# khiner/MeshEditor

Hardware: AMD Instinct MI355X
Metric: eigenpairs/sec (K/M assembly + 50-mode solve, 100k-tet mesh) (higher is better)
Workload: dtype f64; 1 GPU; cube_s100k: Kuhn mesh 105456 tets / 446631 DOF, NumModes=50 NumFemModes=65, P=10 excitation points, one mesh per GPU; eigenpairs_per_mesh=65, kept_modes_per_mesh=50, parallelism=mesh-per-gpu x1

## Files before the change

### mesheditor_amd/csrc/mh_common.h

```cpp
#pragma once
#include "../../include/modalhip.h"

#include <hip/hip_runtime.h>
#include <rocblas/rocblas.h>
#include <rocsolver/rocsolver.h>

#include <algorithm>
#include <cstdarg>
#include <cstdio>
#include <cstdlib>
#include <cstring>
#include <iterator>
#include <limits>
#include <map>
#include <mutex>
#include <stdexcept>
#include <string>
#include <vector>

struct MhError : std::runtime_error {
    int code;
    MhError(int c, const std::string &m) : std::runtime_error(m), code(c) {}
};

// ... 491 lines not shown
    enum Solver { SYEVD = 0, SMALL_PARTIAL = 1, SMALL_STEDC = 2, WIDE_PARTIAL = 3, WIDE_STEDC_ORMTR = 4 };
    int reduction{-1};
    double defect{-1};
    int solver{-1};
    double quality{std::numeric_limits<double>::quiet_NaN()};
};
int mh_rr_solve(mh_context *ctx, double *gA, double *gM, uint32_t m, double *evals, double *ework, DevArray<int> &info, uint32_t nwant = 0, bool gm_is_identity = false,
                std::vector<double> *host_evals = nullptr);
void mh_spd_inverse_small(mh_context *ctx, const double *a, uint32_t lda, uint32_t w, double *out, uint32_t ldo, int *info);
void mh_potrf(mh_context *ctx, double *a, uint32_t ld, uint32_t w, int *info);
void mh_potrf_small(mh_context *ctx, double *a, uint32_t w, int *info);
void mh_potrf_small_inverse(mh_context *ctx, double *a, uint32_t w, int *info, const double *dscale, double *linv);
bool mh_sytrd_gave_up(mh_context *ctx);
void mh_sytrd_wide(mh_context *ctx, double *a, uint32_t m, double *d, double *e, double *tau);
void mh_sytrd_small(mh_context *ctx, double *a, uint32_t m, double *d, double *e, double *tau, int variant = -1);
void mh_small_gemm(mh_context *ctx, bool ta, bool tb, uint32_t M, uint32_t N, uint32_t K, double alpha, const double *a, uint32_t lda, const double *b, uint32_t ldb, double beta, double *c,
                   uint32_t ldc);
void mh_short_product(mh_context *ctx, size_t n, const double *a, uint32_t m, const double *ct, uint32_t nc, double *out, double *partial, uint32_t slices);
void mh_pack_stacked(mh_context *ctx, const double *c1, uint32_t r1, const double *c2, uint32_t r2, uint32_t cols, double scale, double *ct);
void mh_pack_coefficients(mh_context *ctx, const double *c1, uint32_t n1, const double *c2, uint32_t n2, uint32_t m, uint32_t ld, double *ct);
void mh_spmm_mapped(mh_context *ctx, const BsrLevel &lvl, const double *vals9, const double *x, double *y, const double *mscal, double *y2, uint32_t w, uint32_t ldy,
                    uint32_t wreal, const uint32_t *omap, const double *res_theta = nullptr, double *res_out = nullptr, double *res_partial = nullptr,
                    const double *res_dinv = nullptr);
bool mh_spmm_f32_cheb_step(mh_context *ctx, const BsrLevel &lvl, const float *d_in, float *d_out, float *r, float *x, const float *dinv, float c1, float c2,
                           uint32_t w);
void mh_spmm_f32(mh_context *ctx, const BsrLevel &lvl, const float *x, float *y, uint32_t w);
void mh_spmm_mixed(mh_context *ctx, const BsrLevel &lvl, const float *x, double *y, uint32_t w);
const uint32_t *mh_identity_map(mh_context *ctx);
void mh_spmm(mh_context *ctx, const BsrLevel &lvl, const double *vals9, const double *x, double *y, const double *mscal, double *y2, uint32_t w);
```

### mesheditor_amd/csrc/mh_eigs.hip

```cpp
#include "mh_common.h"

#include <algorithm>
#include <cmath>
#include <memory>
#include <condition_variable>
#include <mutex>
#include <numeric>
#include <optional>
#include <type_traits>

__global__ void k_shift_values(const double *kval, const double *mval, size_t nblocks, double sigma, double *aval);
__global__ void k_diag_inverse(const uint32_t *row_ptr, const uint32_t *col, const double *aval, uint32_t nnodes, double *dinv);
__global__ void k_coarse_matrix(const uint32_t *row_ptr, const uint32_t *col, const double *aval, const double *tmat, const uint32_t *agg_of, const uint32_t *agg_ptr,
                                const uint32_t *agg_nodes, uint32_t nagg, double *a0);
__global__ void k_fix_coarse_diag(double *a0, uint32_t n0, double rel);

namespace {
constexpr int TB = 256;

std::mutex g_solve_mutex;
struct Switches {
    bool verbose = getenv("MH_VERBOSE") != nullptr;
    bool fp32_prec = !(getenv("MH_PRECOND_FP64") && atoi(getenv("MH_PRECOND_FP64")) != 0);
    int deg2 = 0, deg1 = 0, gamma = 0;
    double cheb_ratio = 0.0, cheb_ratio1 = 0.0;
    bool test_sytrd_giveup = getenv("MH_TEST") && strstr(getenv("MH_TEST"), "sytrd_giveup");
    bool no_tridiag_wide = getenv("MH_TEST") && strstr(getenv("MH_TEST"), "no_tridiag_wide");
    bool test_last_resort = getenv("MH_TEST") && strstr(getenv("MH_TEST"), "last_resort");
    bool test_coarse_pivot = getenv("MH_TEST") && strstr(getenv("MH_TEST"), "coarse_pivot");
    bool test_selfcheck_fail = getenv("MH_TEST") && strstr(getenv("MH_TEST"), "selfcheck_fail");
    bool lmax_low = getenv("MH_TEST") && strstr(getenv("MH_TEST"), "lmax_low");
    bool potrf_chain = getenv("MH_TEST") && strstr(getenv("MH_TEST"), "potrf_chain");
    bool no_poly_start = getenv("MH_TEST") && strstr(getenv("MH_TEST"), "no_poly_start");
    Switches() {
        if (const char *c = getenv("MH_CYCLE")) {
            double v[5] = {0, 0, 0, 0, 0};
            sscanf(c, "%lf,%lf,%lf,%lf,%lf", &v[0], &v[1], &v[2], &v[3], &v[4]);
            deg2 = std::max(0, int(v[0])), deg1 = std::max(0, int(v[1])), gamma = std::max(0, int(v[2]));
            cheb_ratio = v[3];
            cheb_ratio1 = v[4];
        }
    }
};
const Switches &switches() {
    static const Switches s;
    return s;
}
constexpr int kPowerIterations = 20;
constexpr uint32_t kPrecondColumns = 256;
constexpr uint32_t kSkipP = 4;
constexpr uint32_t kGuardPercent = 10;
constexpr float kFlatShape = 1e-4f;
constexpr size_t kDenseLastResort = 12288;
constexpr int kLastResortCg = 8;

struct PhaseLock {
// ... 71 lines not shown
};

__global__ void k_random_panel(double *__restrict__ x, size_t count, uint64_t seed) {
    const size_t i = size_t(blockIdx.x) * blockDim.x + threadIdx.x;
    if (i >= count) return;
    auto mix = [](uint64_t z) {
        z += 0x9e3779b97f4a7c15ull;
        z = (z ^ (z >> 30)) * 0xbf58476d1ce4e5b9ull;
        z = (z ^ (z >> 27)) * 0x94d049bb133111ebull;
        return z ^ (z >> 31);
    };
    const uint64_t a = mix(seed + 2 * i), b = mix(seed + 2 * i + 1);
    const double u1 = (double(a >> 11) + 1.0) * (1.0 / 9007199254740993.0), u2 = double(b >> 11) * (1.0 / 9007199254740992.0);
    x[i] = sqrt(-2.0 * log(u1)) * cos(6.283185307179586 * u2);
}

template<typename T>
__global__ void k_cheb_init(const T *__restrict__ b, const T *__restrict__ t, const T *__restrict__ dinv, T inv_theta, T *__restrict__ r, T *__restrict__ d,
                            T *__restrict__ x, int accumulate, size_t rows, uint32_t w) {
    const size_t i = size_t(blockIdx.x) * blockDim.x + threadIdx.x;
    if (i >= rows * w) return;
    const T rv = t ? b[i] - t[i] : b[i];
    const T dv = dinv[i / w] * rv * inv_theta;
    r[i] = rv;
    d[i] = dv;
    x[i] = accumulate ? x[i] + dv : dv;
}
typedef float f4_t __attribute__((ext_vector_type(4)));
__global__ void k_cheb_init_v4(const f4_t *__restrict__ b, const f4_t *__restrict__ t, const float *__restrict__ dinv, float inv_theta, f4_t *__restrict__ r,
                               f4_t *__restrict__ d, f4_t *__restrict__ x, int accumulate, size_t rows, uint32_t w4) {
    const size_t i = size_t(blockIdx.x) * blockDim.x + threadIdx.x;
    if (i >= rows * w4) return;
    const f4_t rv = t ? b[i] - t[i] : b[i];
    const f4_t dv = (dinv[i / w4] * inv_theta) * rv;
    r[i] = rv;
    d[i] = dv;
    x[i] = accumulate ? x[i] + dv : dv;
}
__global__ void k_cheb_last_v4(const f4_t *__restrict__ t, const float *__restrict__ dinv, float c1, float c2, const f4_t *__restrict__ r, const f4_t *__restrict__ d,
                               const f4_t *__restrict__ x, double *__restrict__ z, size_t rows, uint32_t w4, uint32_t wo) {
    const size_t i = size_t(blockIdx.x) * blockDim.x + threadIdx.x;
    if (i >= rows * w4) return;
    const size_t row = i / w4;
    const uint32_t c = uint32_t(i % w4) * 4;
    const f4_t rv = r[i] - t[i];
    const f4_t zv = x[i] + (c1 * d[i] + (c2 * dinv[row]) * rv);
#pragma unroll
    for (int e = 0; e < 4; ++e)
        if (c + e < wo) z[row * wo + c + e] = double(zv[e]);
}
__global__ void k_prolong_p1_v4(const f4_t *__restrict__ x1, const uint32_t *__restrict__ pa, const uint32_t *__restrict__ pb, f4_t *__restrict__ x2, uint32_t nnodes,
                                uint32_t w4) {
    const size_t i = size_t(blockIdx.x) * blockDim.x + threadIdx.x;
    if (i >= size_t(nnodes) * 3 * w4) return;
    const uint32_t c = uint32_t(i % w4), comp = uint32_t((i / w4) % 3), node = uint32_t(i / (size_t(3) * w4));
    const uint32_t a = pa[node], bb = pb[node];
    const f4_t va = x1[(size_t(3) * a + comp) * w4 + c];
    x2[i] += a == bb ? va : 0.5f * (va + x1[(size_t(3) * bb + comp) * w4 + c]);
}
__global__ void k_cheb_init_convert(const double *__restrict__ src, uint32_t ws, const float *__restrict__ dinv, float inv_theta, float *__restrict__ b32,
                                    float *__restrict__ r, float *__restrict__ d, float *__restrict__ x, size_t rows, uint32_t w) {
    const size_t i = size_t(blockIdx.x) * blockDim.x + threadIdx.x;
    if (i >= rows * w) return;
    const size_t row = i / w;
    const uint32_t c = uint32_t(i % w);
    const float rv = c < ws ? float(src[row * ws + c]) : 0.f;
    const float dv = dinv[row] * rv * inv_theta;
    b32[i] = rv;
    r[i] = rv;
    d[i] = dv;
    x[i] = dv;
}
template<typename T>
__global__ void k_cheb_step(const T *__restrict__ t, const T *__restrict__ dinv, T c1, T c2, T *__restrict__ r, T *__restrict__ d, T *__restrict__ x, size_t rows,
                            uint32_t w) {
    const size_t i = size_t(blockIdx.x) * blockDim.x + threadIdx.x;
    if (i >= rows * w) return;
    const T rv = r[i] - t[i];
    const T dv = c1 * d[i] + c2 * dinv[i / w] * rv;
    r[i] = rv;
    d[i] = dv;
    x[i] += dv;
}
template<typename T>
__global__ void k_cheb_last(const T *__restrict__ t, const T *__restrict__ dinv, T c1, T c2, const T *__restrict__ r, const T *__restrict__ d, const T *__restrict__ x,
                            double *__restrict__ z, size_t rows, uint32_t w, uint32_t wo) {
    const size_t i = size_t(blockIdx.x) * blockDim.x + threadIdx.x;
    if (i >= rows * w) return;
    const size_t row = i / w;
    const uint32_t c = uint32_t(i % w);
    if (c >= wo) return;
    const T rv = r[i] - t[i];
    z[row * wo + c] = double(x[i] + (c1 * d[i] + c2 * dinv[row] * rv));
}
template<typename S, typename D> __global__ void k_convert(const S *__restrict__ src, D *__restrict__ dst, size_t count) {
    const size_t i = size_t(blockIdx.x) * blockDim.x + threadIdx.x;
    if (i < count) dst[i] = D(src[i]);
}
template<typename S, typename D> __global__ void k_convert_pitch(const S *__restrict__ src, uint32_t ws, D *__restrict__ dst, uint32_t wd, size_t rows) {
    const size_t i = size_t(blockIdx.x) * blockDim.x + threadIdx.x;
    if (i >= rows * wd) return;
    const size_t row = i / wd;
    const uint32_t c = uint32_t(i % wd);
    dst[i] = c < ws ? D(src[row * ws + c]) : D(0);
}

template<typename T>
__global__ void k_restrict_p1(const T *__restrict__ b, const T *__restrict__ t, const uint32_t *__restrict__ p1_corner, const uint32_t *__restrict__ eptr,
                              const uint32_t *__restrict__ emid, T *__restrict__ r1, uint32_t npts, uint32_t w, uint32_t wb = 0) {
    const size_t i = size_t(blockIdx.x) * blockDim.x + threadIdx.x;
    if (i >= size_t(npts) * 3 * w) return;
    const uint32_t c = uint32_t(i % w), comp = uint32_t((i / w) % 3), p = uint32_t(i / (size_t(3) * w));
    const uint32_t pb = wb ? wb : w;
    auto res = [&](uint32_t node) {
        const size_t row = size_t(3) * node + comp;
        return (c < pb ? b[row * pb + c] : T(0)) - t[row * w + c];
    };
    T s = res(p1_corner[p]);
    T h = 0;
    for (uint32_t e = eptr[p]; e < eptr[p + 1]; ++e) h += res(emid[e]);
    r1[i] = s + T(0.5) * h;
}
template<typename T>
__global__ void k_prolong_p1(const T *__restrict__ x1, const uint32_t *__restrict__ pa, const uint32_t *__restrict__ pb, T *__restrict__ x2, uint32_t nnodes,
                             uint32_t w) {
    const size_t i = size_t(blockIdx.x) * blockDim.x + threadIdx.x;
    if (i >= size_t(nnodes) * 3 * w) return;
    const uint32_t c = uint32_t(i % w), comp = uint32_t((i / w) % 3), node = uint32_t(i / (size_t(3) * w));
    const uint32_t a = pa[node], bb = pb[node];
    const T va = x1[(size_t(3) * a + comp) * w + c];
    x2[i] += a == bb ? va : T(0.5) * (va + x1[(size_t(3) * bb + comp) * w + c]);
}
template<typename T>
__global__ void k_restrict_agg(const T *__restrict__ b, const T *__restrict__ t, const double *__restrict__ tmat, double *__restrict__ r0,
                               const uint32_t *__restrict__ agg_ptr, const uint32_t *__restrict__ agg_nodes, uint32_t nagg, uint32_t w) {
    const size_t i = size_t(blockIdx.x) * blockDim.x + threadIdx.x;
    if (i >= size_t(nagg) * 6 * w) return;
    const uint32_t c = uint32_t(i % w), q = uint32_t((i / w) % 6), a = uint32_t(i / (size_t(6) * w));
    double s = 0;
    for (uint32_t l = agg_ptr[a]; l < agg_ptr[a + 1]; ++l) {
        const uint32_t nd = agg_nodes[l];
        const double *tm = tmat + 18 * size_t(nd);
        for (int p = 0; p < 3; ++p) {
            const size_t o = (size_t(3) * nd + p) * w + c;
// ... 556 lines not shown
            rin.reset(ctx, n2 * w);
            t2d.reset(ctx, n2 * w);
            r1d.reset(ctx, n1 * w); t1d.reset(ctx, n1 * w);
        }
        r1.reset(ctx, n1 * w); x1.reset(ctx, n1 * w); d1.reset(ctx, n1 * w); t1.reset(ctx, n1 * w); rr1.reset(ctx, n1 * w);
        r0.reset(ctx, n0 * w);
        x0.reset(ctx, n0 * w);
        x0_partial.reset(ctx, n0 * w * COARSE_SLICES);
        patch_y.reset(ctx, std::max(s->patches2.scratch_rows(), s->patches1.scratch_rows()) * w);
        MhCycleShape shape;
        mh_cycle_shape(s, w_in, &shape);
        deg2 = shape.deg2, deg1 = shape.deg1, gamma = shape.gamma, ratio = shape.ratio, ratio1 = shape.ratio1;
    }
    void spmm(const BsrLevel &lvl, const T *x, T *y, uint32_t w) {
        if constexpr (kDouble) mh_spmm(ctx, lvl, lvl.aval, x, y, nullptr, nullptr, w);
        else mh_spmm_f32(ctx, lvl, x, y, w);
    }
    static const T *dinv_of(const BsrLevel &lvl) {
        if constexpr (kDouble) return lvl.dinv.get();
        else return lvl.dinv32.get();
    }
    const PatchSet &patches_of(const BsrLevel &lvl) const { return lvl.id == 2 ? sys->patches2 : sys->patches1; }
    void cheb(const BsrLevel &lvl, int deg, const T *b, T *x, bool zero_init, T *r, T *d, T *t, uint32_t w, double *z_out = nullptr, uint32_t w_out = 0,
              const double *b_src = nullptr, uint32_t w_src = 0, T *b_copy = nullptr) {
        const size_t rows = size_t(3) * lvl.n_nodes;
        const double lmax = lvl.lmax, lmin = lvl.lmax / (lvl.id == 1 && ratio1 > 0 ? ratio1 : ratio);
        const double theta = 0.5 * (lmax + lmin), delta = 0.5 * (lmax - lmin), sig = theta / delta;
        double rho = 1.0 / sig;
        const T *dinv = dinv_of(lvl);
        if (!zero_init) spmm(lvl, x, t, w);
        if constexpr (!kDouble) {
            if (b_src && zero_init) k_cheb_init_convert<<<grid1(rows * w), TB, 0, ctx->stream>>>(b_src, w_src, dinv, float(1.0 / theta), b_copy, r, d, x, rows, w);
            else k_cheb_init_v4<<<grid1(rows * (w / 4)), TB, 0, ctx->stream>>>(reinterpret_cast<const f4_t *>(b), zero_init ? nullptr : reinterpret_cast<const f4_t *>(t), dinv,
                                                                               float(1.0 / theta), reinterpret_cast<f4_t *>(r), reinterpret_cast<f4_t *>(d),
                                                                               reinterpret_cast<f4_t *>(x), zero_init ? 0 : 1, rows, w / 4);
        } else {
            k_cheb_init<T><<<grid1(rows * w), TB, 0, ctx->stream>>>(b, zero_init ? nullptr : t, dinv, T(1.0 / theta), r, d, x, zero_init ? 0 : 1, rows, w);
        }
        KERNEL_CHECK();
        const PatchSet &ps = patches_of(lvl);
        mh_apply_patches<T>(ctx, ps, r, nullptr, w, T(1.0 / theta), d, x, nullptr, 0, patch_y.get());
        constexpr bool fuse_steps = true;
        T *cur = d, *alt = t;
        for (int k = 1; k < deg; ++k) {
            const double rho_new = 1.0 / (2 * sig - rho);
            const bool last = z_out && k + 1 == deg;
            bool fused = false;
            if constexpr (!kDouble) {
                if (fuse_steps && !last) fused = mh_spmm_f32_cheb_step(ctx, lvl, cur, alt, r, x, dinv, float(rho_new * rho), float(2 * rho_new / delta), w);
            }
            if (fused) {
                std::swap(cur, alt);
                mh_apply_patches<T>(ctx, ps, r, nullptr, w, T(2 * rho_new / delta), cur, x, nullptr, 0, patch_y.get());
            } else {
                spmm(lvl, cur, alt, w);
                if (!last) {
                    k_cheb_step<T><<<grid1(rows * w), TB, 0, ctx->stream>>>(alt, dinv, T(rho_new * rho), T(2 * rho_new / delta), r, cur, x, rows, w);
                } else if constexpr (kDouble) {
                    k_cheb_last<T><<<grid1(rows * w), TB, 0, ctx->stream>>>(alt, dinv, T(rho_new * rho), T(2 * rho_new / delta), r, cur, x, z_out, rows, w, w_out);
                } else {
                    k_cheb_last_v4<<<grid1(rows * (w / 4)), TB, 0, ctx->stream>>>(reinterpret_cast<const f4_t *>(alt), dinv, float(rho_new * rho), float(2 * rho_new / delta),
                                                                             reinterpret_cast<const f4_t *>(r), reinterpret_cast<const f4_t *>(cur),
                                                                             reinterpret_cast<const f4_t *>(x), z_out, rows, w / 4, w_out);
                }
                KERNEL_CHECK();
                if (!last) mh_apply_patches<T>(ctx, ps, r, nullptr, w, T(2 * rho_new / delta), cur, x, nullptr, 0, patch_y.get());
                else mh_apply_patches<T>(ctx, ps, r, alt, w, T(2 * rho_new / delta), nullptr, nullptr, z_out, w_out, patch_y.get());
            }
            rho = rho_new;
        }
        if (z_out && deg == 1) {
            k_convert_pitch<T, double><<<grid1(rows * w_out), TB, 0, ctx->stream>>>(x, w, z_out, w_out, rows);
            KERNEL_CHECK();
        }
    }
    void apply(const double *r_in, double *z_out, uint32_t w_in) {
        mh_finish_hierarchy(sys);
        const uint32_t w = pitch(w_in);
        const uint32_t nn = sys->n_nodes, np = sys->n_points, na = sys->n_agg;
        const size_t n2 = size_t(3) * nn, n1 = size_t(3) * np, n0 = size_t(6) * na;
        const T *r;
        if constexpr (kDouble) r = r_in;
        else r = rin.get();
        T *z = z2.get();
        if constexpr (kDouble) cheb(sys->L2, deg2, r, z, true, r2, d2, t2, w);
        else cheb(sys->L2, deg2, r, z, true, r2, d2, t2, w, nullptr, 0, r_in, w_in, rin.get());
        if constexpr (kDouble) {
            spmm(sys->L2, z, t2, w);
            k_restrict_p1<double><<<grid1(n1 * w), TB, 0, ctx->stream>>>(r, t2.get(), sys->p1_corner, sys->p1_edge_ptr, sys->p1_edge_mid, r1.get(), np, w);
            KERNEL_CHECK();
        } else {
            mh_spmm_mixed(ctx, sys->L2, z, t2d, w);
            k_restrict_p1<double><<<grid1(n1 * w), TB, 0, ctx->stream>>>(r_in, t2d.get(), sys->p1_corner, sys->p1_edge_ptr, sys->p1_edge_mid, r1d.get(), np, w, w_in);
            KERNEL_CHECK();
            k_convert<double, T><<<grid1(n1 * w), TB, 0, ctx->stream>>>(r1d.get(), r1.get(), n1 * w);
            KERNEL_CHECK();
        }
        for (int g = 0; g < gamma; ++g) {
            cheb(sys->L1, deg1, r1, x1, g == 0, rr1, d1, t1, w);
            if constexpr (kDouble) {
                spmm(sys->L1, x1, t1, w);
                k_restrict_agg<double><<<grid1(n0 * w), TB, 0, ctx->stream>>>(r1.get(), t1.get(), sys->agg_t, r0, sys->agg_ptr, sys->agg_nodes, na, w);
            } else {
                mh_spmm_mixed(ctx, sys->L1, x1, t1d, w);
                k_restrict_agg<double><<<grid1(n0 * w), TB, 0, ctx->stream>>>(r1d.get(), t1d.get(), sys->agg_t, r0, sys->agg_ptr, sys->agg_nodes, na, w);
            }
            KERNEL_CHECK();
            mh_short_product(ctx, n0, sys->a0, uint32_t(n0), r0, w, x0, x0_partial, COARSE_SLICES);
            k_prolong_agg<T><<<grid1(n1 * w), TB, 0, ctx->stream>>>(x0, sys->agg_t, x1.get(), sys->agg_of, np, w);
            KERNEL_CHECK();
            cheb(sys->L1, deg1, r1, x1, false, rr1, d1, t1, w);
        }
        if constexpr (kDouble) k_prolong_p1<T><<<grid1(n2 * w), TB, 0, ctx->stream>>>(x1.get(), sys->parent_a, sys->parent_b, z, nn, w);
        else k_prolong_p1_v4<<<grid1(n2 * (w / 4)), TB, 0, ctx->stream>>>(reinterpret_cast<const f4_t *>(x1.get()), sys->parent_a, sys->parent_b, reinterpret_cast<f4_t *>(z), nn, w / 4);
        KERNEL_CHECK();
        cheb(sys->L2, deg2, r, z, false, r2, d2, t2, w, z_out, w_in);
    }
};

// ... 655 lines not shown
            best_worst_active = std::min(best_worst_active, worst_active);
            hist_active.push_back(worst_active);
            if (inner_cg > 0 && it >= 40) {
                const size_t h = hist_active.size();
                if (h > 30 && hist_nconv[h - 31] == nconv && worst_active > 0.9 * hist_active[h - 31] && worst_active <= 10.0 * residual_tol) {
                    pairs_at_floor = nev > nconv ? nev - nconv : 0;
                    if (verbose) fprintf(stderr, "[lobpcg] it %3u: %u pairs have sat at a residual of %.2e (tolerance %.1e) for thirty iterations -- the rounding floor of this mesh; handed on as they are\n", it, pairs_at_floor, worst_active, residual_tol);
                    converged = true;
                    return true;
                }
            }
            floor_strikes = it >= 20 && worst_active > 1e3 * best_worst_active ? floor_strikes + 1 : 0;
            if (floor_strikes >= 3)
                mh_throw(MH_ENOTCONVERGED, "LOBPCG: %u of %u pairs converged; the others sit at the rounding floor (residual %.1e and growing, best %.1e, tolerance %.1e)", nconv, nev,
                         worst_active, best_worst_active, residual_tol);
        }
        return false;
    }

    void search_directions(uint32_t it) {
        w = uint32_t(act.size());
        idx_d.upload(act.data(), w);
        const double *residuals = Rw.get();
        if (rw_from_rr) {
            if (act == res_act && res_pitch == w) {
                residuals = Rr.get();
            } else {
                std::vector<uint32_t> &pos = res_pos;
                pos.assign(w, 0);
                size_t q = 0;
                for (uint32_t k = 0; k < w; ++k) {
                    while (q < res_act.size() && res_act[q] != act[k]) ++q;
                    if (q == res_act.size()) mh_throw(MH_EHIP, "active column %u was not active before", act[k]);
                    pos[k] = uint32_t(q);
                }
                pos_d.upload(pos.data(), w);
                k_gather_cols<<<grid1(n * w), TB, 0, st>>>(Rr, pos_d, Rw, n, res_pitch, w);
                KERNEL_CHECK();
            }
        } else {
            k_gather_cols<<<grid1(n * w), TB, 0, st>>>(R, idx_d, Rw, n, b, w);
            KERNEL_CHECK();
        }
        for (uint32_t k = 0; k < w; ++k) theta_act[k] = theta[act[k]];
        theta_act_d.upload(theta_act.data(), w);
        {
            Timer tp(ctx);
            precondition(residuals, W, w);
            precond_seconds += tp.stop();
            prof.op_applications += w;
        }
        bool ok = true;
        p_implicit = false;
        if (pproj_ok && wp) {
            gram(ctx, n, MX, b, W, w, H, b);
            mh_pack_stacked(ctx, H, b, nullptr, 0, w, -1.0, Ct);
            mh_combine(ctx, n, X, b, nullptr, 0, nullptr, 0, Ct, w, W, w, nullptr, true);
            mh_spmm(ctx, sys->L2, sys->L2.aval, W, AW, sys->L2.mval, MW, w);
            gram(ctx, n, P, wp, MW, w, Hp, wp);
            lazy_images = true;
            w_implicit = false;
            ok = chol_orthonormalise(W, MW, AW, w, false, true, Hp, wp);
            if (!ok) mh_throw(MH_ENOTCONVERGED, "search directions lost rank at iteration %u", it);
            if (p_needs_explicit) {
                mh_pack_stacked(ctx, Hp, wp, nullptr, 0, w, -1.0, Ct);
                mh_combine(ctx, n, P, wp, nullptr, 0, nullptr, 0, Ct, w, W, w, nullptr, true);
                mh_spmm(ctx, sys->L2, sys->L2.aval, W, AW, sys->L2.mval, MW, w);
                lazy_images = w <= 256;
                ok = chol_orthonormalise(W, MW, AW, w, !lazy_images, lazy_images);
                if (!ok) mh_throw(MH_ENOTCONVERGED, "search directions lost rank at iteration %u", it);
            } else {
// ... 467 lines not shown
```

### mesheditor_amd/csrc/mh_spmm.hip

```cpp
#include "mh_common.h"

namespace {
#ifndef MH_SPMM_TB
#define MH_SPMM_TB 64
#endif
constexpr int TB = MH_SPMM_TB;
#ifndef MH_SPMM_U
#define MH_SPMM_U 1
#endif

template<typename T, int CW, int NC, bool WITH_M, bool WITH_A>
__global__ void __launch_bounds__(TB) k_spmm(const uint32_t *__restrict__ row_ptr, const uint32_t *__restrict__ col, const T *__restrict__ vals9,
                                            const T *__restrict__ mscal, const T *__restrict__ x, T *__restrict__ y, T *__restrict__ y2,
                                            uint32_t nnodes, uint32_t w, int xcd_remap) {
    constexpr int RPW = 64 / CW;
    const int lane = threadIdx.x & 63, wave = threadIdx.x >> 6;
    const uint32_t c0 = blockIdx.y * (CW * NC) + (lane % CW);
    const uint32_t nb = gridDim.x, per = (nb + 7) / 8;
    const uint32_t bid = xcd_remap ? (blockIdx.x % 8) * per + blockIdx.x / 8 : blockIdx.x;
    uint32_t row = (bid * (TB / 64) + wave) * RPW + lane / CW;
    if (RPW == 1) row = __builtin_amdgcn_readfirstlane(row);
    if (row >= nnodes) return;
    bool active[NC];
    uint32_t cc[NC];
// ... 45 lines not shown
                if (WITH_M) {
                    m0[k] += m[u] * x0;
                    m1[k] += m[u] * x1;
                    m2[k] += m[u] * x2;
                }
            }
        }
        p += U;
    };
    constexpr int UMAX = NC >= 3 ? 2 : (NC == 2 ? 4 : 8);
    while (p + UMAX <= p1) step(std::integral_constant<int, UMAX>{});
    if (UMAX >= 8 && p + 4 <= p1) step(std::integral_constant<int, 4>{});
    if (UMAX >= 4 && p + 2 <= p1) step(std::integral_constant<int, 2>{});
    while (p < p1) step(std::integral_constant<int, 1>{});
#pragma unroll
    for (int k = 0; k < NC; ++k) {
        if (!active[k]) continue;
        const size_t o = size_t(3) * row * w + c0 + CW * k;
        if (WITH_A) { y[o] = a0[k]; y[o + w] = a1[k]; y[o + 2 * size_t(w)] = a2[k]; }
        if (WITH_M) { y2[o] = m0[k]; y2[o + w] = m1[k]; y2[o + 2 * size_t(w)] = m2[k]; }
    }
}

struct ChebStep {
    float *r = nullptr;
    const float *dinv = nullptr;
    float *d_out = nullptr;
    float *x = nullptr;
    float c1 = 0.f, c2 = 0.f;
};
struct ResidualEpilogue {
    const double *theta = nullptr;
    double *r_out = nullptr;
    double *partial = nullptr;
    const double *dinv = nullptr;
};
#ifdef MH_SPMM_WAVES
#define MH_SPMM_OCC __attribute__((amdgpu_waves_per_eu(MH_SPMM_WAVES, 8)))
#else
#define MH_SPMM_OCC
#endif
template<typename TV, typename TX, typename TY, int V, int CL, bool WITH_M, bool WITH_A, bool MAPOUT = false, int EPI = 0, int UR = MH_SPMM_U, bool PRE = false>
__global__ void __launch_bounds__(TB) MH_SPMM_OCC k_spmm_wide(const uint32_t *__restrict__ row_ptr, const uint32_t *__restrict__ col, const TV *__restrict__ vals9,
                                                 const TV *__restrict__ mscal, const TX *__restrict__ x, TY *__restrict__ y, TY *__restrict__ y2, uint32_t nnodes,
                                                 uint32_t w, int xcd_remap, uint32_t ldy = 0, uint32_t wreal = 0, const uint32_t *__restrict__ omap = nullptr, ChebStep epi = ChebStep{},
                                                 uint32_t xpitch = 0, ResidualEpilogue res = ResidualEpilogue{}) {
    constexpr int G = 64 / CL, STRIP = 64, VP = sizeof(TV) == 4 ? 12 : 10, U = UR;
    typedef TX Vec __attribute__((ext_vector_type(V)));
    typedef TY Acc __attribute__((ext_vector_type(V)));
    __shared__ __attribute__((aligned(16))) TV sv[TB / 64][WITH_A ? (STRIP + 1) * VP : 1];
    __shared__ TV sm[TB / 64][WITH_M ? STRIP + 1 : 1];
    __shared__ uint32_t sc[TB / 64][STRIP + 1];
    const int lane = threadIdx.x & 63, wave = threadIdx.x >> 6;
    const uint32_t c = lane % CL, g = lane / CL;
    const uint32_t nb_grid = gridDim.x, per = (nb_grid + 7) / 8;
    const uint32_t bid = xcd_remap ? (blockIdx.x % 8) * per + blockIdx.x / 8 : blockIdx.x;
    const uint32_t row = __builtin_amdgcn_readfirstlane(bid * (TB / 64) + wave);
    if (row >= nnodes) return;
    const bool act = V * c < w && g < G;
    const uint32_t coff = act ? V * c : 0;
    Acc acc[3], macc[3];
#pragma unroll
    for (int i = 0; i < 3; ++i) acc[i] = macc[i] = Acc(0);
    Acc er[PRE ? 3 : 1], ed[PRE ? 3 : 1], ex[PRE ? 3 : 1];
    TY edinv[PRE ? 3 : 1];
    if constexpr (EPI == 1 && PRE) {
        if (g == 0 && act) {
            const size_t o = size_t(3) * row * w + coff;
#pragma unroll
            for (int i = 0; i < 3; ++i) {
                er[i] = *reinterpret_cast<const Acc *>(epi.r + o + size_t(i) * w);
                ed[i] = __builtin_convertvector(*reinterpret_cast<const Vec *>(x + o + size_t(i) * w), Acc);
                ex[i] = *reinterpret_cast<const Acc *>(epi.x + o + size_t(i) * w);
                edinv[i] = epi.dinv[size_t(3) * row + i];
            }
        }
    }
    const uint32_t p0 = __builtin_amdgcn_readfirstlane(row_ptr[row]), p1 = __builtin_amdgcn_readfirstlane(row_ptr[row + 1]);
    TV *svw = sv[wave];
    TV *smw = sm[wave];
    uint32_t *scw = sc[wave];
    for (uint32_t base = p0; base < p1; base += STRIP) {
        const uint32_t nb = min(uint32_t(STRIP), p1 - base);
        if (base != p0) __builtin_amdgcn_fence(__ATOMIC_ACQ_REL, "wavefront");
        scw[lane] = uint32_t(lane) < nb ? col[base + lane] : 0u;
        if (WITH_A) {
            const TV *src = vals9 + size_t(9) * base;
            TV tmp[9];
#pragma unroll
            for (int i = 0; i < 9; ++i) {
                const uint32_t f = lane + 64 * i;
                tmp[i] = f < 9 * nb ? src[f] : TV(0);
            }
#pragma unroll
            for (int i = 0; i < 9; ++i) {
                const uint32_t f = lane + 64 * i;
// ... 58 lines not shown
        }
    } else {
#pragma unroll
        for (int i = 0; i < 3; ++i) {
#pragma unroll
            for (int e = 0; e < V; ++e) {
                TY sa = acc[i][e], sm_ = macc[i][e];
#pragma unroll
                for (int j = 1; j < G; ++j) {
                    if (WITH_A) sa += __shfl_down(acc[i][e], j * CL, 64);
                    if (WITH_M) sm_ += __shfl_down(macc[i][e], j * CL, 64);
                }
                acc[i][e] = sa;
                macc[i][e] = sm_;
            }
        }
    }
    if constexpr (EPI == 1) {
        if (g == 0 && act) {
            const size_t o = size_t(3) * row * w + coff;
#pragma unroll
            for (int i = 0; i < 3; ++i) {
                const size_t oi = o + size_t(i) * w;
                Acc rv, dv, xn;
                if constexpr (PRE) {
                    rv = er[i] - acc[i];
                    dv = epi.c1 * ed[i] + (epi.c2 * edinv[i]) * rv;
                    xn = ex[i] + dv;
                } else {
                    rv = *reinterpret_cast<const Acc *>(epi.r + oi) - acc[i];
                    dv = epi.c1 * __builtin_convertvector(*reinterpret_cast<const Vec *>(x + oi), Acc) + (epi.c2 * epi.dinv[size_t(3) * row + i]) * rv;
                    xn = *reinterpret_cast<const Acc *>(epi.x + oi) + dv;
                }
                *reinterpret_cast<Acc *>(epi.r + oi) = rv;
                *reinterpret_cast<Acc *>(epi.d_out + oi) = dv;
                *reinterpret_cast<Acc *>(epi.x + oi) = xn;
            }
        }
        return;
    }
    if (MAPOUT) {
        if (g == 0 && act) {
#pragma unroll
            for (int e = 0; e < V; ++e) {
                if (coff + e >= wreal) continue;
                const size_t o = size_t(3) * row * ldy + omap[coff + e];
                if (WITH_A) { y[o] = acc[0][e]; y[o + ldy] = acc[1][e]; y[o + 2 * size_t(ldy)] = acc[2][e]; }
                if (WITH_M) { y2[o] = macc[0][e]; y2[o + ldy] = macc[1][e]; y2[o + 2 * size_t(ldy)] = macc[2][e]; }
            }
            if constexpr (WITH_A && WITH_M && std::is_same<TY, double>::value && V == 2) {
                if (res.r_out) {
                    Acc th, sr = Acc(0), sm = Acc(0);
                    th[0] = res.theta[coff];
                    th[1] = res.theta[coff + 1];
#pragma unroll
                    for (int i = 0; i < 3; ++i) {
                        const Acc r = acc[i] - th * macc[i];
                        const TY wgt = res.dinv ? res.dinv[size_t(3) * row + i] : TY(1);
// ... 132 lines not shown
        mh_throw(MH_EINVAL, "residual epilogue needs a panel of at most 128 columns (got %u)", w);
    }
    if (w % 2 || (reinterpret_cast<uintptr_t>(x) & 15)) mh_throw(MH_EINVAL, "mapped product needs an even pitch and an aligned panel (got %u)", w);
    constexpr int xcd = 1;
    const unsigned grid = (div_up(lvl.n_nodes, TB / 64) + 7) / 8 * 8;
    const uint32_t ranges = div_up(w, 128u), step = (div_up(w, ranges) + 1u) & ~1u;
    for (uint32_t c0 = 0; c0 < wreal; c0 += step) {
        const uint32_t wc = std::min(step, w - c0), wr = std::min(wc, wreal - c0);
        TimedLaunch timed(ctx, MH_KERNEL_SPMM, spmm_bytes(lvl, wr, 8, 8, 8, true, true) + (res.r_out ? 8.0 * double(wr) * (3.0 + 2.0) * double(lvl.n_nodes) : 0.0));
        auto go = [&](auto cl_tag) {
            constexpr int CL = decltype(cl_tag)::value;
            k_spmm_wide<double, double, double, 2, CL, true, true, true><<<grid, TB, 0, ctx->stream>>>(lvl.row_ptr, lvl.col, vals9, mscal, x + c0, y, y2, lvl.n_nodes, wc, xcd, ldy, wr, omap + c0,
                                                                                                  ChebStep{}, w, res);
        };
        const uint32_t lanes = wc / 2;
        if (lanes <= 8) go(std::integral_constant<int, 8>{});
        else if (lanes <= 16) go(std::integral_constant<int, 16>{});
        else if (lanes <= 32) go(std::integral_constant<int, 32>{});
        else go(std::integral_constant<int, 64>{});
        KERNEL_CHECK();
    }
}

bool mh_spmm_f32_cheb_step(mh_context *ctx, const BsrLevel &lvl, const float *d_in, float *d_out, float *r, float *x, const float *dinv, float c1, float c2, uint32_t w) {
    if (w == 0) return true;
    const bool aligned16 = !((reinterpret_cast<uintptr_t>(d_in) | reinterpret_cast<uintptr_t>(d_out) | reinterpret_cast<uintptr_t>(r) | reinterpret_cast<uintptr_t>(x)) & 15);
    if (w % 4 || w > 256 || !aligned16) return false;
    TimedLaunch timed(ctx, MH_KERNEL_SPMM, spmm_bytes(lvl, w, 4, 4, 0, true, false) + 5.0 * 4.0 * 3.0 * double(lvl.n_nodes) * w);
    constexpr int xcd = 1;
    const unsigned grid = (div_up(lvl.n_nodes, TB / 64) + 7) / 8 * 8;
    ChebStep epi;
    epi.r = r; epi.dinv = dinv; epi.d_out = d_out; epi.x = x; epi.c1 = c1; epi.c2 = c2;
    auto go = [&](auto cl_tag) {
        constexpr int CL = decltype(cl_tag)::value;
        if (latency_bound_level(lvl))
            k_spmm_wide<float, float, float, 4, CL, false, true, false, 1, 4, true><<<grid, TB, 0, ctx->stream>>>(lvl.row_ptr, lvl.col, lvl.aval32.get(), static_cast<const float *>(nullptr), d_in,
                                                                                                                static_cast<float *>(nullptr), static_cast<float *>(nullptr), lvl.n_nodes, w, xcd, 0, 0, nullptr, epi);
        else
            k_spmm_wide<float, float, float, 4, CL, false, true, false, 1><<<grid, TB, 0, ctx->stream>>>(lvl.row_ptr, lvl.col, lvl.aval32.get(), static_cast<const float *>(nullptr), d_in,
                                                                                                       static_cast<float *>(nullptr), static_cast<float *>(nullptr), lvl.n_nodes, w, xcd, 0, 0, nullptr, epi);
    };
    const uint32_t lanes = w / 4;
    if (lanes <= 8) go(std::integral_constant<int, 8>{});
    else if (lanes <= 16) go(std::integral_constant<int, 16>{});
    else if (lanes <= 20) go(std::integral_constant<int, 20>{});
    else if (lanes <= 32) go(std::integral_constant<int, 32>{});
    else go(std::integral_constant<int, 64>{});
    KERNEL_CHECK();
    return true;
}

void mh_spmm_f32(mh_context *ctx, const BsrLevel &lvl, const float *x, float *y, uint32_t w) {
    if (w == 0) return;
    TimedLaunch timed(ctx, MH_KERNEL_SPMM, spmm_bytes(lvl, w, 4, 4, 4, true, false));
    launch_spmm<float, false, true>(ctx, lvl, lvl.aval32.get(), x, y, static_cast<const float *>(nullptr), static_cast<float *>(nullptr), w);
// ... 9 lines not shown
```

Baseline: 617.0 eigenpairs/s.

## Elide redundant Chebyshev smoother stores and gather-free residual input

The Chebyshev smoother now skips writing r and x on the first step of a cold start (x equals d, r equals b) and skips storing d/r on the final step, controlled by mode flags threaded through the fused SpMM epilogue and the elementwise kernels. The fp32 preconditioner reads residual columns directly through a column map instead of gathering them into a contiguous panel, and restriction writes the fp32 copy directly, dropping a separate convert kernel. Together these cut memory traffic in the multigrid smoother at the cost of more mode-dependent branching and explicit FMA ordering that may change rounding slightly.

```diff
diff --git a/mesheditor_amd/csrc/mh_common.h b/mesheditor_amd/csrc/mh_common.h
--- a/mesheditor_amd/csrc/mh_common.h
+++ b/mesheditor_amd/csrc/mh_common.h
@@ -537,8 +537,9 @@
 void mh_spmm_mapped(mh_context *ctx, const BsrLevel &lvl, const double *vals9, const double *x, double *y, const double *mscal, double *y2, uint32_t w, uint32_t ldy,
                     uint32_t wreal, const uint32_t *omap, const double *res_theta = nullptr, double *res_out = nullptr, double *res_partial = nullptr,
                     const double *res_dinv = nullptr);
+enum : unsigned { MH_CHEB_X_IS_D = 1u, MH_CHEB_ADD_D = 2u, MH_CHEB_KEEP_R = 4u, MH_CHEB_KEEP_D = 8u };
 bool mh_spmm_f32_cheb_step(mh_context *ctx, const BsrLevel &lvl, const float *d_in, float *d_out, float *r, float *x, const float *dinv, float c1, float c2,
-                           uint32_t w);
+                           uint32_t w, const float *r_in = nullptr, unsigned mode = MH_CHEB_KEEP_R | MH_CHEB_KEEP_D);
 void mh_spmm_f32(mh_context *ctx, const BsrLevel &lvl, const float *x, float *y, uint32_t w);
 void mh_spmm_mixed(mh_context *ctx, const BsrLevel &lvl, const float *x, double *y, uint32_t w);
 const uint32_t *mh_identity_map(mh_context *ctx);
diff --git a/mesheditor_amd/csrc/mh_eigs.hip b/mesheditor_amd/csrc/mh_eigs.hip
--- a/mesheditor_amd/csrc/mh_eigs.hip
+++ b/mesheditor_amd/csrc/mh_eigs.hip
@@ -32,6 +32,7 @@
     bool lmax_low = getenv("MH_TEST") && strstr(getenv("MH_TEST"), "lmax_low");
     bool potrf_chain = getenv("MH_TEST") && strstr(getenv("MH_TEST"), "potrf_chain");
     bool no_poly_start = getenv("MH_TEST") && strstr(getenv("MH_TEST"), "no_poly_start");
+    bool smoother_all_passes = getenv("MH_TEST") && strstr(getenv("MH_TEST"), "smoother_all_passes");
     Switches() {
         if (const char *c = getenv("MH_CYCLE")) {
             double v[5] = {0, 0, 0, 0, 0};
@@ -149,9 +150,9 @@
     if (i >= rows * w) return;
     const T rv = t ? b[i] - t[i] : b[i];
     const T dv = dinv[i / w] * rv * inv_theta;
-    r[i] = rv;
+    if (r) r[i] = rv;
     d[i] = dv;
-    x[i] = accumulate ? x[i] + dv : dv;
+    if (x) x[i] = accumulate ? x[i] + dv : dv;
 }
 typedef float f4_t __attribute__((ext_vector_type(4)));
 __global__ void k_cheb_init_v4(const f4_t *__restrict__ b, const f4_t *__restrict__ t, const float *__restrict__ dinv, float inv_theta, f4_t *__restrict__ r,
@@ -160,18 +161,30 @@
     if (i >= rows * w4) return;
     const f4_t rv = t ? b[i] - t[i] : b[i];
     const f4_t dv = (dinv[i / w4] * inv_theta) * rv;
-    r[i] = rv;
+    if (r) r[i] = rv;
     d[i] = dv;
-    x[i] = accumulate ? x[i] + dv : dv;
+    if (x) x[i] = accumulate ? x[i] + dv : dv;
+}
+template<typename V, typename S> __device__ __forceinline__ V cheb_direction(S c1, V d, S s, V r) {
+#pragma clang fp contract(off)
+    const V a = c1 * d, b = s * r;
+    return a + b;
+}
+__device__ __forceinline__ double cheb_direction(double c1, double d, double s, double r) {
+#pragma clang fp contract(off)
+    return __builtin_fma(c1, d, s * r);
 }
 __global__ void k_cheb_last_v4(const f4_t *__restrict__ t, const float *__restrict__ dinv, float c1, float c2, const f4_t *__restrict__ r, const f4_t *__restrict__ d,
-                               const f4_t *__restrict__ x, double *__restrict__ z, size_t rows, uint32_t w4, uint32_t wo) {
+                               const f4_t *__restrict__ x, double *__restrict__ z, size_t rows, uint32_t w4, uint32_t wo, unsigned mode) {
     const size_t i = size_t(blockIdx.x) * blockDim.x + threadIdx.x;
     if (i >= rows * w4) return;
     const size_t row = i / w4;
     const uint32_t c = uint32_t(i % w4) * 4;
     const f4_t rv = r[i] - t[i];
-    const f4_t zv = x[i] + (c1 * d[i] + (c2 * dinv[row]) * rv);
+    const f4_t dc = d[i];
+    f4_t xb = mode & MH_CHEB_X_IS_D ? dc : x[i];
+    if (mode & MH_CHEB_ADD_D) xb = xb + dc;
+    const f4_t zv = xb + cheb_direction(c1, dc, c2 * dinv[row], rv);
 #pragma unroll
     for (int e = 0; e < 4; ++e)
         if (c + e < wo) z[row * wo + c + e] = double(zv[e]);
@@ -186,39 +199,46 @@
     x2[i] += a == bb ? va : 0.5f * (va + x1[(size_t(3) * bb + comp) * w4 + c]);
 }
 __global__ void k_cheb_init_convert(const double *__restrict__ src, uint32_t ws, const float *__restrict__ dinv, float inv_theta, float *__restrict__ b32,
-                                    float *__restrict__ r, float *__restrict__ d, float *__restrict__ x, size_t rows, uint32_t w) {
+                                    float *__restrict__ r, float *__restrict__ d, float *__restrict__ x, size_t rows, uint32_t w, uint32_t ld_src,
+                                    const uint32_t *__restrict__ cmap) {
     const size_t i = size_t(blockIdx.x) * blockDim.x + threadIdx.x;
     if (i >= rows * w) return;
     const size_t row = i / w;
     const uint32_t c = uint32_t(i % w);
-    const float rv = c < ws ? float(src[row * ws + c]) : 0.f;
+    const float rv = c < ws ? float(src[row * ld_src + (cmap ? cmap[c] : c)]) : 0.f;
     const float dv = dinv[row] * rv * inv_theta;
     b32[i] = rv;
-    r[i] = rv;
+    if (r) r[i] = rv;
     d[i] = dv;
-    x[i] = dv;
+    if (x) x[i] = dv;
 }
 template<typename T>
-__global__ void k_cheb_step(const T *__restrict__ t, const T *__restrict__ dinv, T c1, T c2, T *__restrict__ r, T *__restrict__ d, T *__restrict__ x, size_t rows,
-                            uint32_t w) {
+__global__ void k_cheb_step(const T *__restrict__ t, const T *__restrict__ dinv, T c1, T c2, const T *r_in, T *r, T *__restrict__ d, T *__restrict__ x, size_t rows,
+                            uint32_t w, unsigned mode) {
     const size_t i = size_t(blockIdx.x) * blockDim.x + threadIdx.x;
     if (i >= rows * w) return;
-    const T rv = r[i] - t[i];
-    const T dv = c1 * d[i] + c2 * dinv[i / w] * rv;
-    r[i] = rv;
-    d[i] = dv;
-    x[i] += dv;
+    const T rv = r_in[i] - t[i];
+    const T dc = d[i];
+    T xb = mode & MH_CHEB_X_IS_D ? dc : x[i];
+    if (mode & MH_CHEB_ADD_D) xb = xb + dc;
+    const T dv = cheb_direction(c1, dc, c2 * dinv[i / w], rv);
+    if (mode & MH_CHEB_KEEP_R) r[i] = rv;
+    if (mode & MH_CHEB_KEEP_D) d[i] = dv;
+    x[i] = xb + dv;
 }
 template<typename T>
 __global__ void k_cheb_last(const T *__restrict__ t, const T *__restrict__ dinv, T c1, T c2, const T *__restrict__ r, const T *__restrict__ d, const T *__restrict__ x,
-                            double *__restrict__ z, size_t rows, uint32_t w, uint32_t wo) {
+                            double *__restrict__ z, size_t rows, uint32_t w, uint32_t wo, unsigned mode) {
     const size_t i = size_t(blockIdx.x) * blockDim.x + threadIdx.x;
     if (i >= rows * w) return;
     const size_t row = i / w;
     const uint32_t c = uint32_t(i % w);
     if (c >= wo) return;
     const T rv = r[i] - t[i];
-    z[row * wo + c] = double(x[i] + (c1 * d[i] + c2 * dinv[row] * rv));
+    const T dc = d[i];
+    T xb = mode & MH_CHEB_X_IS_D ? dc : x[i];
+    if (mode & MH_CHEB_ADD_D) xb = xb + dc;
+    z[row * wo + c] = double(xb + cheb_direction(c1, dc, c2 * dinv[row], rv));
 }
 template<typename S, typename D> __global__ void k_convert(const S *__restrict__ src, D *__restrict__ dst, size_t count) {
     const size_t i = size_t(blockIdx.x) * blockDim.x + threadIdx.x;
@@ -234,19 +254,22 @@
 
 template<typename T>
 __global__ void k_restrict_p1(const T *__restrict__ b, const T *__restrict__ t, const uint32_t *__restrict__ p1_corner, const uint32_t *__restrict__ eptr,
-                              const uint32_t *__restrict__ emid, T *__restrict__ r1, uint32_t npts, uint32_t w, uint32_t wb = 0) {
+                              const uint32_t *__restrict__ emid, T *__restrict__ r1, uint32_t npts, uint32_t w, uint32_t wb = 0, float *__restrict__ r1s = nullptr,
+                              uint32_t ldb = 0, const uint32_t *__restrict__ bmap = nullptr) {
     const size_t i = size_t(blockIdx.x) * blockDim.x + threadIdx.x;
     if (i >= size_t(npts) * 3 * w) return;
     const uint32_t c = uint32_t(i % w), comp = uint32_t((i / w) % 3), p = uint32_t(i / (size_t(3) * w));
-    const uint32_t pb = wb ? wb : w;
+    const uint32_t nb = wb ? wb : w, pb = ldb ? ldb : nb, cb = bmap && c < nb ? bmap[c] : c;
     auto res = [&](uint32_t node) {
         const size_t row = size_t(3) * node + comp;
-        return (c < pb ? b[row * pb + c] : T(0)) - t[row * w + c];
+        return (c < nb ? b[row * pb + cb] : T(0)) - t[row * w + c];
     };
     T s = res(p1_corner[p]);
     T h = 0;
     for (uint32_t e = eptr[p]; e < eptr[p + 1]; ++e) h += res(emid[e]);
-    r1[i] = s + T(0.5) * h;
+    const T v = s + T(0.5) * h;
+    r1[i] = v;
+    if (r1s) r1s[i] = float(v);
 }
 template<typename T>
 __global__ void k_prolong_p1(const T *__restrict__ x1, const uint32_t *__restrict__ pa, const uint32_t *__restrict__ pb, T *__restrict__ x2, uint32_t nnodes,
@@ -849,50 +872,56 @@
     }
     const PatchSet &patches_of(const BsrLevel &lvl) const { return lvl.id == 2 ? sys->patches2 : sys->patches1; }
     void cheb(const BsrLevel &lvl, int deg, const T *b, T *x, bool zero_init, T *r, T *d, T *t, uint32_t w, double *z_out = nullptr, uint32_t w_out = 0,
-              const double *b_src = nullptr, uint32_t w_src = 0, T *b_copy = nullptr) {
+              const double *b_src = nullptr, uint32_t w_src = 0, T *b_copy = nullptr, uint32_t ld_src = 0, const uint32_t *map_src = nullptr) {
         const size_t rows = size_t(3) * lvl.n_nodes;
         const double lmax = lvl.lmax, lmin = lvl.lmax / (lvl.id == 1 && ratio1 > 0 ? ratio1 : ratio);
         const double theta = 0.5 * (lmax + lmin), delta = 0.5 * (lmax - lmin), sig = theta / delta;
         double rho = 1.0 / sig;
         const T *dinv = dinv_of(lvl);
+        const PatchSet &ps = patches_of(lvl);
+        const bool all = switches().smoother_all_passes, patched = ps.n_patches || ps.n_clusters;
+        const bool cold_defer = !all && zero_init && deg >= 2, warm_defer = !all && !zero_init && deg >= 2 && !patched;
+        T *r_init = cold_defer ? nullptr : r, *x_init = cold_defer || warm_defer ? nullptr : x;
         if (!zero_init) spmm(lvl, x, t, w);
         if constexpr (!kDouble) {
-            if (b_src && zero_init) k_cheb_init_convert<<<grid1(rows * w), TB, 0, ctx->stream>>>(b_src, w_src, dinv, float(1.0 / theta), b_copy, r, d, x, rows, w);
+            if (b_src && zero_init) k_cheb_init_convert<<<grid1(rows * w), TB, 0, ctx->stream>>>(b_src, w_src, dinv, float(1.0 / theta), b_copy, r_init, d, x_init, rows, w, map_src ? ld_src : w_src, map_src);
             else k_cheb_init_v4<<<grid1(rows * (w / 4)), TB, 0, ctx->stream>>>(reinterpret_cast<const f4_t *>(b), zero_init ? nullptr : reinterpret_cast<const f4_t *>(t), dinv,
-                                                                               float(1.0 / theta), reinterpret_cast<f4_t *>(r), reinterpret_cast<f4_t *>(d),
-                                                                               reinterpret_cast<f4_t *>(x), zero_init ? 0 : 1, rows, w / 4);
+                                                                               float(1.0 / theta), reinterpret_cast<f4_t *>(r_init), reinterpret_cast<f4_t *>(d),
+                                                                               reinterpret_cast<f4_t *>(x_init), zero_init ? 0 : 1, rows, w / 4);
         } else {
-            k_cheb_init<T><<<grid1(rows * w), TB, 0, ctx->stream>>>(b, zero_init ? nullptr : t, dinv, T(1.0 / theta), r, d, x, zero_init ? 0 : 1, rows, w);
+            k_cheb_init<T><<<grid1(rows * w), TB, 0, ctx->stream>>>(b, zero_init ? nullptr : t, dinv, T(1.0 / theta), r_init, d, x_init, zero_init ? 0 : 1, rows, w);
         }
         KERNEL_CHECK();
-        const PatchSet &ps = patches_of(lvl);
-        mh_apply_patches<T>(ctx, ps, r, nullptr, w, T(1.0 / theta), d, x, nullptr, 0, patch_y.get());
+        mh_apply_patches<T>(ctx, ps, cold_defer ? b : r, nullptr, w, T(1.0 / theta), d, x_init, nullptr, 0, patch_y.get());
         constexpr bool fuse_steps = true;
         T *cur = d, *alt = t;
         for (int k = 1; k < deg; ++k) {
             const double rho_new = 1.0 / (2 * sig - rho);
-            const bool last = z_out && k + 1 == deg;
+            const bool final_step = k + 1 == deg, last = z_out && final_step;
+            const T *r_src = k == 1 && cold_defer ? b : r;
+            const bool keep_d = all || !final_step, keep_r = keep_d || patched;
+            const unsigned mode = (k == 1 && cold_defer ? MH_CHEB_X_IS_D : 0u) | (k == 1 && warm_defer ? MH_CHEB_ADD_D : 0u) | (keep_r ? MH_CHEB_KEEP_R : 0u) | (keep_d ? MH_CHEB_KEEP_D : 0u);
             bool fused = false;
             if constexpr (!kDouble) {
-                if (fuse_steps && !last) fused = mh_spmm_f32_cheb_step(ctx, lvl, cur, alt, r, x, dinv, float(rho_new * rho), float(2 * rho_new / delta), w);
+                if (fuse_steps && !last) fused = mh_spmm_f32_cheb_step(ctx, lvl, cur, alt, r, x, dinv, float(rho_new * rho), float(2 * rho_new / delta), w, r_src, mode);
             }
             if (fused) {
                 std::swap(cur, alt);
-                mh_apply_patches<T>(ctx, ps, r, nullptr, w, T(2 * rho_new / delta), cur, x, nullptr, 0, patch_y.get());
+                mh_apply_patches<T>(ctx, ps, r, nullptr, w, T(2 * rho_new / delta), keep_d ? cur : nullptr, x, nullptr, 0, patch_y.get());
             } else {
                 spmm(lvl, cur, alt, w);
                 if (!last) {
-                    k_cheb_step<T><<<grid1(rows * w), TB, 0, ctx->stream>>>(alt, dinv, T(rho_new * rho), T(2 * rho_new / delta), r, cur, x, rows, w);
+                    k_cheb_step<T><<<grid1(rows * w), TB, 0, ctx->stream>>>(alt, dinv, T(rho_new * rho), T(2 * rho_new / delta), r_src, r, cur, x, rows, w, mode);
                 } else if constexpr (kDouble) {
-                    k_cheb_last<T><<<grid1(rows * w), TB, 0, ctx->stream>>>(alt, dinv, T(rho_new * rho), T(2 * rho_new / delta), r, cur, x, z_out, rows, w, w_out);
+                    k_cheb_last<T><<<grid1(rows * w), TB, 0, ctx->stream>>>(alt, dinv, T(rho_new * rho), T(2 * rho_new / delta), r_src, cur, x, z_out, rows, w, w_out, mode);
                 } else {
                     k_cheb_last_v4<<<grid1(rows * (w / 4)), TB, 0, ctx->stream>>>(reinterpret_cast<const f4_t *>(alt), dinv, float(rho_new * rho), float(2 * rho_new / delta),
-                                                                             reinterpret_cast<const f4_t *>(r), reinterpret_cast<const f4_t *>(cur),
-                                                                             reinterpret_cast<const f4_t *>(x), z_out, rows, w / 4, w_out);
+                                                                             reinterpret_cast<const f4_t *>(r_src), reinterpret_cast<const f4_t *>(cur),
+                                                                             reinterpret_cast<const f4_t *>(x), z_out, rows, w / 4, w_out, mode);
                 }
                 KERNEL_CHECK();
-                if (!last) mh_apply_patches<T>(ctx, ps, r, nullptr, w, T(2 * rho_new / delta), cur, x, nullptr, 0, patch_y.get());
-                else mh_apply_patches<T>(ctx, ps, r, alt, w, T(2 * rho_new / delta), nullptr, nullptr, z_out, w_out, patch_y.get());
+                if (!last) mh_apply_patches<T>(ctx, ps, r, nullptr, w, T(2 * rho_new / delta), keep_d ? cur : nullptr, x, nullptr, 0, patch_y.get());
+                else mh_apply_patches<T>(ctx, ps, r_src, alt, w, T(2 * rho_new / delta), nullptr, nullptr, z_out, w_out, patch_y.get());
             }
             rho = rho_new;
         }
@@ -901,7 +930,8 @@
             KERNEL_CHECK();
         }
     }
-    void apply(const double *r_in, double *z_out, uint32_t w_in) {
+    void apply(const double *r_in, double *z_out, uint32_t w_in, uint32_t ld_in = 0, const uint32_t *cmap = nullptr) {
+        if (kDouble && cmap) mh_throw(MH_EINVAL, "the double-precision cycle takes a contiguous panel");
         mh_finish_hierarchy(sys);
         const uint32_t w = pitch(w_in);
         const uint32_t nn = sys->n_nodes, np = sys->n_points, na = sys->n_agg;
@@ -911,17 +941,20 @@
         else r = rin.get();
         T *z = z2.get();
         if constexpr (kDouble) cheb(sys->L2, deg2, r, z, true, r2, d2, t2, w);
-        else cheb(sys->L2, deg2, r, z, true, r2, d2, t2, w, nullptr, 0, r_in, w_in, rin.get());
+        else cheb(sys->L2, deg2, r, z, true, r2, d2, t2, w, nullptr, 0, r_in, w_in, rin.get(), ld_in, cmap);
         if constexpr (kDouble) {
             spmm(sys->L2, z, t2, w);
             k_restrict_p1<double><<<grid1(n1 * w), TB, 0, ctx->stream>>>(r, t2.get(), sys->p1_corner, sys->p1_edge_ptr, sys->p1_edge_mid, r1.get(), np, w);
             KERNEL_CHECK();
         } else {
             mh_spmm_mixed(ctx, sys->L2, z, t2d, w);
-            k_restrict_p1<double><<<grid1(n1 * w), TB, 0, ctx->stream>>>(r_in, t2d.get(), sys->p1_corner, sys->p1_edge_ptr, sys->p1_edge_mid, r1d.get(), np, w, w_in);
-            KERNEL_CHECK();
-            k_convert<double, T><<<grid1(n1 * w), TB, 0, ctx->stream>>>(r1d.get(), r1.get(), n1 * w);
-            KERNEL_CHECK();
+            const bool all = switches().smoother_all_passes;
+            k_restrict_p1<double><<<grid1(n1 * w), TB, 0, ctx->stream>>>(r_in, t2d.get(), sys->p1_corner, sys->p1_edge_ptr, sys->p1_edge_mid, r1d.get(), np, w, w_in, all ? nullptr : r1.get(), cmap ? ld_in : 0, cmap);
+            KERNEL_CHECK();
+            if (all) {
+                k_convert<double, T><<<grid1(n1 * w), TB, 0, ctx->stream>>>(r1d.get(), r1.get(), n1 * w);
+                KERNEL_CHECK();
+            }
         }
         for (int g = 0; g < gamma; ++g) {
             cheb(sys->L1, deg1, r1, x1, g == 0, rr1, d1, t1, w);
@@ -1623,6 +1656,9 @@
         w = uint32_t(act.size());
         idx_d.upload(act.data(), w);
         const double *residuals = Rw.get();
+        const bool in_place = prec32 && !panel_cg && w <= kPrecondColumns && !switches().smoother_all_passes;
+        const uint32_t *res_map = nullptr;
+        uint32_t res_ld = 0;
         if (rw_from_rr) {
             if (act == res_act && res_pitch == w) {
                 residuals = Rr.get();
@@ -1636,9 +1672,15 @@
                     pos[k] = uint32_t(q);
                 }
                 pos_d.upload(pos.data(), w);
-                k_gather_cols<<<grid1(n * w), TB, 0, st>>>(Rr, pos_d, Rw, n, res_pitch, w);
-                KERNEL_CHECK();
-            }
+                if (in_place) {
+                    residuals = Rr.get(), res_ld = res_pitch, res_map = pos_d.get();
+                } else {
+                    k_gather_cols<<<grid1(n * w), TB, 0, st>>>(Rr, pos_d, Rw, n, res_pitch, w);
+                    KERNEL_CHECK();
+                }
+            }
+        } else if (in_place) {
+            residuals = R.get(), res_ld = b, res_map = idx_d.get();
         } else {
             k_gather_cols<<<grid1(n * w), TB, 0, st>>>(R, idx_d, Rw, n, b, w);
             KERNEL_CHECK();
@@ -1647,7 +1689,8 @@
         theta_act_d.upload(theta_act.data(), w);
         {
             Timer tp(ctx);
-            precondition(residuals, W, w);
+            if (res_map) prec32->apply(residuals, W, w, res_ld, res_map);
+            else precondition(residuals, W, w);
             precond_seconds += tp.stop();
             prof.op_applications += w;
         }
diff --git a/mesheditor_amd/csrc/mh_spmm.hip b/mesheditor_amd/csrc/mh_spmm.hip
--- a/mesheditor_amd/csrc/mh_spmm.hip
+++ b/mesheditor_amd/csrc/mh_spmm.hip
@@ -91,12 +91,19 @@
     }
 }
 
+template<typename A, typename S> __device__ __forceinline__ A cheb_fused_direction(S c1, A d, S s, A r) {
+#pragma clang fp contract(off)
+    const A m = s * r;
+    return __builtin_elementwise_fma(A(c1), d, m);
+}
 struct ChebStep {
+    const float *r_in = nullptr;
     float *r = nullptr;
     const float *dinv = nullptr;
     float *d_out = nullptr;
     float *x = nullptr;
     float c1 = 0.f, c2 = 0.f;
+    unsigned mode = MH_CHEB_KEEP_R | MH_CHEB_KEEP_D;
 };
 struct ResidualEpilogue {
     const double *theta = nullptr;
@@ -138,9 +145,9 @@
             const size_t o = size_t(3) * row * w + coff;
 #pragma unroll
             for (int i = 0; i < 3; ++i) {
-                er[i] = *reinterpret_cast<const Acc *>(epi.r + o + size_t(i) * w);
+                er[i] = *reinterpret_cast<const Acc *>(epi.r_in + o + size_t(i) * w);
                 ed[i] = __builtin_convertvector(*reinterpret_cast<const Vec *>(x + o + size_t(i) * w), Acc);
-                ex[i] = *reinterpret_cast<const Acc *>(epi.x + o + size_t(i) * w);
+                ex[i] = epi.mode & MH_CHEB_X_IS_D ? ed[i] : *reinterpret_cast<const Acc *>(epi.x + o + size_t(i) * w);
                 edinv[i] = epi.dinv[size_t(3) * row + i];
             }
         }
@@ -245,18 +252,24 @@
 #pragma unroll
             for (int i = 0; i < 3; ++i) {
                 const size_t oi = o + size_t(i) * w;
-                Acc rv, dv, xn;
+                Acc rv, dc, xb;
+                TY di;
                 if constexpr (PRE) {
                     rv = er[i] - acc[i];
-                    dv = epi.c1 * ed[i] + (epi.c2 * edinv[i]) * rv;
-                    xn = ex[i] + dv;
+                    dc = ed[i];
+                    xb = ex[i];
+                    di = edinv[i];
                 } else {
-                    rv = *reinterpret_cast<const Acc *>(epi.r + oi) - acc[i];
-                    dv = epi.c1 * __builtin_convertvector(*reinterpret_cast<const Vec *>(x + oi), Acc) + (epi.c2 * epi.dinv[size_t(3) * row + i]) * rv;
-                    xn = *reinterpret_cast<const Acc *>(epi.x + oi) + dv;
-                }
-                *reinterpret_cast<Acc *>(epi.r + oi) = rv;
-                *reinterpret_cast<Acc *>(epi.d_out + oi) = dv;
+                    rv = *reinterpret_cast<const Acc *>(epi.r_in + oi) - acc[i];
+                    dc = __builtin_convertvector(*reinterpret_cast<const Vec *>(x + oi), Acc);
+                    xb = epi.mode & MH_CHEB_X_IS_D ? dc : *reinterpret_cast<const Acc *>(epi.x + oi);
+                    di = epi.dinv[size_t(3) * row + i];
+                }
+                if (epi.mode & MH_CHEB_ADD_D) xb = xb + dc;
+                const Acc dv = cheb_fused_direction(TY(epi.c1), dc, TY(epi.c2) * di, rv);
+                const Acc xn = xb + dv;
+                if (epi.mode & MH_CHEB_KEEP_R) *reinterpret_cast<Acc *>(epi.r + oi) = rv;
+                if (epi.mode & MH_CHEB_KEEP_D) *reinterpret_cast<Acc *>(epi.d_out + oi) = dv;
                 *reinterpret_cast<Acc *>(epi.x + oi) = xn;
             }
         }
@@ -435,15 +448,19 @@
     }
 }
 
-bool mh_spmm_f32_cheb_step(mh_context *ctx, const BsrLevel &lvl, const float *d_in, float *d_out, float *r, float *x, const float *dinv, float c1, float c2, uint32_t w) {
+bool mh_spmm_f32_cheb_step(mh_context *ctx, const BsrLevel &lvl, const float *d_in, float *d_out, float *r, float *x, const float *dinv, float c1, float c2, uint32_t w,
+                           const float *r_in, unsigned mode) {
     if (w == 0) return true;
-    const bool aligned16 = !((reinterpret_cast<uintptr_t>(d_in) | reinterpret_cast<uintptr_t>(d_out) | reinterpret_cast<uintptr_t>(r) | reinterpret_cast<uintptr_t>(x)) & 15);
+    if (!r_in) r_in = r;
+    const bool aligned16 =
+        !((reinterpret_cast<uintptr_t>(d_in) | reinterpret_cast<uintptr_t>(d_out) | reinterpret_cast<uintptr_t>(r) | reinterpret_cast<uintptr_t>(x) | reinterpret_cast<uintptr_t>(r_in)) & 15);
     if (w % 4 || w > 256 || !aligned16) return false;
-    TimedLaunch timed(ctx, MH_KERNEL_SPMM, spmm_bytes(lvl, w, 4, 4, 0, true, false) + 5.0 * 4.0 * 3.0 * double(lvl.n_nodes) * w);
+    const int passes = 2 + (mode & MH_CHEB_X_IS_D ? 0 : 1) + (mode & MH_CHEB_KEEP_R ? 1 : 0) + (mode & MH_CHEB_KEEP_D ? 1 : 0);
+    TimedLaunch timed(ctx, MH_KERNEL_SPMM, spmm_bytes(lvl, w, 4, 4, 0, true, false) + passes * 4.0 * 3.0 * double(lvl.n_nodes) * w);
     constexpr int xcd = 1;
     const unsigned grid = (div_up(lvl.n_nodes, TB / 64) + 7) / 8 * 8;
     ChebStep epi;
-    epi.r = r; epi.dinv = dinv; epi.d_out = d_out; epi.x = x; epi.c1 = c1; epi.c2 = c2;
+    epi.r_in = r_in; epi.r = r; epi.dinv = dinv; epi.d_out = d_out; epi.x = x; epi.c1 = c1; epi.c2 = c2; epi.mode = mode;
     auto go = [&](auto cl_tag) {
         constexpr int CL = decltype(cl_tag)::value;
         if (latency_bound_level(lvl))
```

New measurement: 634.7 eigenpairs/s (median of 6 runs). 1.03x the previous value.
